# CognitiveAISystems/MAPF-GPT

Measured on AMD Instinct MI355X. Metric: agent-steps/s (env+obs+GPT fwd), higher is better.
Workload: dtype f16x3

## Files before the change

mapf_gpt_amd/csrc/gpt_kernels_attn_tiles.h:

```cpp
#pragma once
#include "gpt_kernels_c256p.h"

namespace mgpt {
namespace fastk {

constexpr int kAttNvb1 = 10, kAttNvb2 = 6;

__device__ unsigned long long g_attn_fallbacks = 0;

template <class T, int NP, int KROW, int VROW, int HS>
__device__ __forceinline__ void attention_exact_tiles(unsigned kr_addr, unsigned vr_addr, const u32x4 (&qf)[2][2], float sc2, f32x16 &o, float &l_run)
{
    float m_run, zero;
    asm volatile("v_mov_b32 %0, 0xff800000\n\tv_mov_b32 %1, 0" : "=v"(m_run), "=v"(zero));
    l_run = zero;
#pragma unroll
    for (int g = 0; g < 16; g++) o[g] = zero;
{
    u32x4 kf[2][2], vf[2][2];
    auto load_k = [&](int kt) {
        const unsigned a = kr_addr + (unsigned)kt * (32 * KROW);
        asm volatile("ds_read_b128 %0, %1" : "=v"(kf[0][0]) : "v"(a) : "memory");
        asm volatile("ds_read_b128 %0, %1 offset:32" : "=v"(kf[1][0]) : "v"(a) : "memory");
        if (NP == 2) {
            asm volatile("ds_read_b128 %0, %1 offset:%2" : "=v"(kf[0][1]) : "v"(a), "n"(kT * KROW) : "memory");
            asm volatile("ds_read_b128 %0, %1 offset:%2" : "=v"(kf[1][1]) : "v"(a), "n"(kT * KROW + 32) : "memory");
        } else { kf[0][1] = kf[0][0]; kf[1][1] = kf[1][0]; }
    };
    load_k(0);
#pragma unroll 1
    for (int kt = 0; kt < kT / 32; kt++) {
        f32x16 sc;
#pragma unroll
        for (int g = 0; g < 16; g++) sc[g] = 0.f;
        asm volatile("s_waitcnt lgkmcnt(0)" ::: "memory");
        __builtin_amdgcn_sched_barrier(0);
#pragma unroll
        for (int ks = 0; ks < 2; ks++) sc = mma<T, NP>(kf[ks], qf[ks], sc);
        __builtin_amdgcn_sched_barrier(0);
        {
            const unsigned a = vr_addr + (unsigned)kt * 64;
            asm volatile("ds_read_b128 %0, %1" : "=v"(vf[0][0]) : "v"(a) : "memory");
            asm volatile("ds_read_b128 %0, %1 offset:32" : "=v"(vf[1][0]) : "v"(a) : "memory");
            if (NP == 2) {
                asm volatile("ds_read_b128 %0, %1 offset:%2" : "=v"(vf[0][1]) : "v"(a), "n"(HS * VROW) : "memory");
                asm volatile("ds_read_b128 %0, %1 offset:%2" : "=v"(vf[1][1]) : "v"(a), "n"(HS * VROW + 32) : "memory");
            } else { vf[0][1] = vf[0][0]; vf[1][1] = vf[1][0]; }
        }
        if (kt + 1 < kT / 32) load_k(kt + 1);
        float mx = sc[0];
#pragma unroll
        for (int g = 1; g < 16; g++) mx = fmaxf(mx, sc[g]);
        mx = other_half_max(mx);
        if (__builtin_amdgcn_ballot_w64(mx > m_run) != 0) {
            const float m_new = fmaxf(m_run, mx);
            const float alpha = __builtin_amdgcn_exp2f((m_run - m_new) * sc2);
            l_run *= alpha;
#pragma unroll
            for (int g = 0; g < 16; g++) o[g] *= alpha;
            m_run = m_new;
        }
        const float nm = -m_run * sc2;
        float psum = 0.f;
#pragma unroll
        for (int g = 0; g < 16; g++) {
            sc[g] = __builtin_amdgcn_exp2f(fmaf(sc[g], sc2, nm));
            psum += sc[g];
        }
        l_run += other_half_sum(psum);
        u32x4 pf[2][2];
#pragma unroll
        for (int mm = 0; mm < 2; mm++) pack_octet<T, NP>(sc, mm, pf[mm]);
        if (kt + 1 < kT / 32) asm volatile("s_waitcnt lgkmcnt(%0)" ::"n"(2 * NP) : "memory");
        else asm volatile("s_waitcnt lgkmcnt(0)" ::: "memory");
        __builtin_amdgcn_sched_barrier(0);
#pragma unroll
        for (int mm = 0; mm < 2; mm++) o = mma<T, NP>(vf[mm], pf[mm], o);
    }
}
}

template <class T, int NP, int KROW, int VROW, int HS>
__device__ __forceinline__ void attention_tiles(unsigned kr_addr, unsigned vr_addr, const u32x4 (&qf)[2][2], int lane, f32x16 &o, float &l_run)
{
    using I0 = std::integral_constant<int, 0>;
    using I1 = std::integral_constant<int, 1>;

    u32x4 kf[2][2], vf[2][2], pf[2][2];
    f32x16 sA, sB;
    constexpr int NM = NP == 2 ? 3 : 1;
    auto amfma = [&](u32x4 a, u32x4 b2, f32x16 c) { return T::mfma(a, b2, c); };
    auto amma = [&](const u32x4 (&a)[2], const u32x4 (&b2)[2], f32x16 c) {
        if (NP == 2) { c = amfma(a[1], b2[0], c); c = amfma(a[0], b2[1], c); }
        return amfma(a[0], b2[0], c);
    };
    auto load_k = [&](auto kt_c) {
        constexpr int off = decltype(kt_c)::value * (32 * KROW);
        asm volatile("ds_read_b128 %0, %1 offset:%2" : "=v"(kf[0][0]) : "v"(kr_addr), "n"(off) : "memory");
        asm volatile("ds_read_b128 %0, %1 offset:%2" : "=v"(kf[1][0]) : "v"(kr_addr), "n"(off + 32) : "memory");
        if (NP == 2) {
            asm volatile("ds_read_b128 %0, %1 offset:%2" : "=v"(kf[0][1]) : "v"(kr_addr), "n"(off + kT * KROW) : "memory");
            asm volatile("ds_read_b128 %0, %1 offset:%2" : "=v"(kf[1][1]) : "v"(kr_addr), "n"(off + kT * KROW + 32) : "memory");
        } else { kf[0][1] = kf[0][0]; kf[1][1] = kf[1][0]; }
    };
    auto load_v = [&](auto kt_c, auto mm_c) {
        constexpr int off = decltype(kt_c)::value * 64 + decltype(mm_c)::value * 32, mm = decltype(mm_c)::value;
        asm volatile("ds_read_b128 %0, %1 offset:%2" : "=v"(vf[mm][0]) : "v"(vr_addr), "n"(off) : "memory");
        if (NP == 2) asm volatile("ds_read_b128 %0, %1 offset:%2" : "=v"(vf[mm][1]) : "v"(vr_addr), "n"(off + HS * VROW) : "memory");
        else vf[mm][1] = vf[mm][0];
    };
    auto lgkm = [&](auto n_c) {
        asm volatile("s_waitcnt lgkmcnt(%0)" ::"n"(decltype(n_c)::value) : "memory");
        __builtin_amdgcn_sched_barrier(0);
    };
    auto place = [&](auto nmf_c, auto nv_c) {
#pragma unroll
        for (int n = 0; n < decltype(nmf_c)::value; n++) {
            __builtin_amdgcn_sched_group_barrier(0x008, 1, 0);
            __builtin_amdgcn_sched_group_barrier(0x002, decltype(nv_c)::value, 0);
        }
        __builtin_amdgcn_sched_group_barrier(0x002, 64, 0);
        __builtin_amdgcn_sched_barrier(0);
    };
    using LK = std::integral_constant<int, 2 * NP>;
    using LV = std::integral_constant<int, NP>;
    load_k(I0{});
    lgkm(I0{});
#pragma unroll
    for (int g = 0; g < 16; g++) sA[g] = 0.f;
#pragma unroll
    for (int ks = 0; ks < 2; ks++) sA = amma(kf[ks], qf[ks], sA);
    __builtin_amdgcn_sched_barrier(0);
    load_k(I1{});
    f32x16 nmb;
    {
        float mx = sA[0];
#pragma unroll
        for (int g = 1; g < 16; g++) mx = fmaxf(mx, sA[g]);
        const float nm = -other_half_max(mx);
#pragma unroll
        for (int g = 0; g < 16; g++) { nmb[g] = nm; sA[g] += nm; }
    }
    float l_part = 0.f;
    auto tile = [&](auto kt_c, f32x16 &cur, f32x16 &nxt) {
        constexpr int kt = decltype(kt_c)::value;
        constexpr bool FIRSTT = kt == 0, LASTT = kt == kT / 32 - 1, HAS2 = kt + 2 < kT / 32;
        if constexpr (!FIRSTT) {
            lgkm(std::integral_constant<int, LASTT ? 0 : LK::value>{});
            o = amma(vf[1], pf[1], o);
#pragma unroll
            for (int g = 0; g < 4; g++) {
                cur[g] = __builtin_amdgcn_exp2f(cur[g]);
                l_part += cur[g];
            }
            place(std::integral_constant<int, NM>{}, std::integral_constant<int, 4>{});
            asm volatile("" : "+v"(o));
        }
        load_v(kt_c, I0{});
        if constexpr (!LASTT) {
            lgkm(LV{});
            nxt = amma(kf[0], qf[0], nmb);
            nxt = amma(kf[1], qf[1], nxt);
        }
#pragma unroll
        for (int g = FIRSTT ? 0 : 4; g < 16; g++) {
            cur[g] = __builtin_amdgcn_exp2f(cur[g]);
            l_part += cur[g];
        }
        pack_octet<T, NP>(cur, 0, pf[0]);
        place(std::integral_constant<int, LASTT ? 0 : 2 * NM>{}, std::integral_constant<int, kAttNvb1>{});
        if constexpr (!LASTT) asm volatile("" : "+v"(nxt));
        load_v(kt_c, I1{});
        lgkm(LV{});
        if constexpr (FIRSTT) {
#pragma unroll
            for (int g = 0; g < 16; g++) o[g] = 0.f;
        }
        o = amma(vf[0], pf[0], o);
        pack_octet<T, NP>(cur, 1, pf[1]);
        place(std::integral_constant<int, NM>{}, std::integral_constant<int, kAttNvb2>{});
        asm volatile("" : "+v"(o));
        if constexpr (HAS2) load_k(std::integral_constant<int, HAS2 ? kt + 2 : 0>{});
    };
    using K0 = std::integral_constant<int, 0>; using K1 = std::integral_constant<int, 1>; using K2 = std::integral_constant<int, 2>; using K3 = std::integral_constant<int, 3>;
    using K4 = std::integral_constant<int, 4>; using K5 = std::integral_constant<int, 5>; using K6 = std::integral_constant<int, 6>; using K7 = std::integral_constant<int, 7>;
    static_assert(kT / 32 == 8, "eight key tiles");
    tile(K0{}, sA, sB); tile(K1{}, sB, sA); tile(K2{}, sA, sB); tile(K3{}, sB, sA);
    tile(K4{}, sA, sB); tile(K5{}, sB, sA); tile(K6{}, sA, sB); tile(K7{}, sB, sA);
    lgkm(I0{});
    o = amma(vf[1], pf[1], o);
    __builtin_amdgcn_sched_barrier(0);
    l_run = other_half_sum(l_part);
    if (__builtin_amdgcn_ballot_w64(!(l_part < 60000.0f)) != 0) {
        if (lane == 0) atomicAdd(&g_attn_fallbacks, 1ull);
        attention_exact_tiles<T, NP, KROW, VROW, HS>(kr_addr, vr_addr, qf, 1.0f, o, l_run);
    }
}

}
}
```

mapf_gpt_amd/csrc/gpt_kernels_c256b.h:

```cpp
#pragma once
#include "gpt_kernels_c256p.h"
#include "gpt_kernels_attn_tiles.h"

namespace mgpt {
namespace fastk {

constexpr int kA256oProjSteps = 16;
constexpr int kA256oPeriod = 8 * kA256StepsPerHead + kA256oProjSteps;


template <class T, int NP>
__global__ __launch_bounds__(256) void pack_attn256q_kernel(const float *__restrict__ w_attn, const float *__restrict__ gain,
                                                            const float *__restrict__ w_proj, uint16_t *__restrict__ out,
                                                            float scale_a, float scale_p)
{
    constexpr int C = 256, NH = 8, QKV = NH * kA256StepsPerHead;
    const int64_t gid = (int64_t)blockIdx.x * 256 + threadIdx.x;
    if (gid >= (int64_t)kA256oPeriod * 8 * 64) return;
    const int lane = (int)(gid & 63), ms = (int)((gid >> 6) & 7), G = (int)(gid >> 9);
    const int rho = lane & 15, qk = lane >> 4;
    float v[8];
    if (G < QKV) {
        const int head = G / kA256StepsPerHead, st = G - head * kA256StepsPerHead;
        int which, kb, dim;
        if (st < 4) {
            const int cc = 4 * st + (ms >> 1), ug = ms & 1, rq = rho >> 2;
            kb = cc >> 1; which = cc & 1;
            const int blk = which == 0 ? 2 * (rq & 1) + (rq >> 1) : rq;
            dim = 8 * blk + 4 * ug + (rho & 3);
        } else { which = 2; kb = 4 * (st - 4) + (ms >> 1); dim = 16 * (ms & 1) + rho; }
        const float *row = w_attn + (size_t)(which * C + head * 32 + dim) * C;
#pragma unroll
        for (int e = 0; e < 8; e++) {
            const int col = 32 * kb + 8 * qk + e;
            v[e] = row[col] * gain[col] * scale_a;
        }
    } else {
        const int s = G - QKV, tt = s >> 2, j = s & 3;
        const int cc = 4 * j + (ms >> 1), kb = cc >> 1, fgl = 2 * (cc & 1) + (ms & 1);
        const float *row = w_proj + (size_t)(64 * tt + 16 * fgl + rho) * C;
#pragma unroll
        for (int e = 0; e < 8; e++) {
            const int col = 32 * kb + (e & 3) + 8 * (2 * (qk & 1) + (e >> 2)) + 4 * (qk >> 1);
            v[e] = row[col] * scale_p;
        }
    }
    u32x2 h0, l0, h1, l1;
    split4<T, NP>(v, h0, l0);
    split4<T, NP>(v + 4, h1, l1);
    u32x4 hi, lo;
    hi[0] = h0[0]; hi[1] = h0[1]; hi[2] = h1[0]; hi[3] = h1[1];
    lo[0] = l0[0]; lo[1] = l0[1]; lo[2] = l1[0]; lo[3] = l1[1];
    uint16_t *dst = out + (((size_t)G * 8 + ms) * NP) * 512 + (size_t)lane * 8;
    *reinterpret_cast<u32x4 *>(dst) = hi;
    if (NP == 2) *reinterpret_cast<u32x4 *>(dst + 512) = lo;
}

template <int NP> constexpr int kL0TabHeadBytes = 192 * NP;
template <int NP> constexpr int kL0TabEntryBytes = 8 * kL0TabHeadBytes<NP>;
template <class T, int NP, bool EMB = false, int TAB = 0>
__global__ __launch_bounds__(512, 2) void attn256q_kernel(float *__restrict__ x, const uint16_t *__restrict__ wstream, float inv_scale,
                                                          float scale_log2e, float inv_proj, unsigned char *__restrict__ spill,
                                                          int n_rows, const unsigned char *__restrict__ tokens = nullptr,
                                                          const float *__restrict__ etab = nullptr, unsigned char *__restrict__ table = nullptr)
{
    static_assert(TAB == 0 || (TAB == 1 && EMB) || (TAB == 2 && !EMB), "table modes");
    constexpr int HB = kL0TabHeadBytes<NP>, ENT = kL0TabEntryBytes<NP>;
    constexpr int C = 256, KS = 16, NH = 8, HS = 32, NW = 8;
    static_assert(NP == 2 || NP == 1, "planes");
    constexpr int MS = 8;
    constexpr int STEP = MS * NP * 1024;
    constexpr int NSLOT = 5;
    constexpr int PW = MS * NP / NW;
    constexpr int KROW = 80, VROW = 528;
    constexpr int NSPILL = 2 * NP;
    constexpr int NYLD = 14 * NP;
    static_assert(PW >= 1, "a wave moves at least one piece per step");
    extern __shared__ __attribute__((aligned(16))) unsigned char smem[];
    const int tid = threadIdx.x, lane = tid & 63;
    const int wave = __builtin_amdgcn_readfirstlane(tid >> 6);
    const int tok0 = wave * 32;
    const unsigned lane16 = (unsigned)lane * 16u;
    const unsigned lds0 = (unsigned)(size_t)smem + lane16;
    const unsigned sK = (unsigned)(size_t)smem + NSLOT * STEP, sV = sK + NP * kT * KROW;
    constexpr int PERIOD = TAB == 2 ? kA256oProjSteps : kA256oPeriod;
    const unsigned char *wbase = reinterpret_cast<const unsigned char *>(wstream) + (size_t)(wave * PW) * 1024 +
                                 (TAB == 2 ? (size_t)(kA256oPeriod - kA256oProjSteps) * STEP : 0);
    unsigned char *sp_wave = spill + ((size_t)blockIdx.x * NW + wave) * (size_t)(14 * NP * 1024);
    const int n_mine = n_rows > (int)blockIdx.x ? (n_rows - 1 - (int)blockIdx.x) / (int)gridDim.x + 1 : 0;
    if (n_mine == 0) return;

    int r_issue = 0;
    int slot_cur = 0, slot_prev = NSLOT - 1;
    unsigned cur_addr = 0, nxt_addr = 0;
    auto issue = [&](int slot) {
        const unsigned char *src = wbase + (size_t)r_issue * STEP;
        unsigned char *dst = smem + (size_t)slot * STEP + (size_t)(wave * PW) * 1024;
#pragma unroll
        for (int i = 0; i < PW; i++) dma_piece(src + lane16, dst, std::integral_constant<int, 0>{}, i);
        r_issue = r_issue + 1 == PERIOD ? 0 : r_issue + 1;
    };
#pragma unroll
    for (int G = 0; G < NSLOT - 1; G++) issue(G);
    auto sync_wait = [&](auto pending_c) {
        vm_wait<decltype(pending_c)::value>();
        __builtin_amdgcn_s_barrier();
    };
    int slot_refill = 0;
    auto sync_issue = [&]() {
        issue(slot_prev);
        const int slot_next = slot_cur + 1 == NSLOT ? 0 : slot_cur + 1;
        cur_addr = lds0 + (unsigned)slot_cur * STEP;
        nxt_addr = lds0 + (unsigned)slot_next * STEP;
        slot_prev = slot_cur;
        slot_cur = slot_next;
    };
    u32x4 wb[2][2][2];
    auto chunk_wait = [&]() {
        asm volatile("s_waitcnt lgkmcnt(0)" ::: "memory");
        __builtin_amdgcn_sched_barrier(0);
    };
    auto chunk_read = [&](auto c_c, auto next_c, auto n_c) {
        constexpr int c = decltype(c_c)::value, n = decltype(n_c)::value;
        if constexpr (n < 2 * NP) {
            constexpr int fr = n / NP, pl = n % NP;
            if constexpr (c < 3) lds_frag(cur_addr, std::integral_constant<int, ((2 * c + 2 + fr) * NP + pl) * 1024>{}, wb[(c + 1) & 1][fr][pl]);
            else if constexpr (decltype(next_c)::value) lds_frag(nxt_addr, std::integral_constant<int, (fr * NP + pl) * 1024>{}, wb[0][fr][pl]);
            if constexpr (NP == 1 && (c < 3 || decltype(next_c)::value)) wb[(c + 1) & 1][fr][1] = wb[(c + 1) & 1][fr][0];
            __builtin_amdgcn_sched_barrier(0);
        }
    };
    using I0 = std::integral_constant<int, 0>;
    using I1 = std::integral_constant<int, 1>;
    using I2 = std::integral_constant<int, 2>;
    using I3 = std::integral_constant<int, 3>;
    auto mma4 = [&](const u32x4 (&w0)[2], const u32x4 (&w1)[2], const u32x4 (&x0)[2], const u32x4 (&x1)[2], f32x16 &blk, auto swap_c, auto first_c, auto &&behind) {
        constexpr bool SW = decltype(swap_c)::value, FIRST = decltype(first_c)::value;
        auto one = [&](const u32x4 &w, const u32x4 &xx, auto s_c) {
            if constexpr (SW) mm16<T>(xx, w, blk, s_c); else mm16<T>(w, xx, blk, s_c);
        };
        auto onez = [&](const u32x4 &w, const u32x4 &xx, auto s_c) {
            if constexpr (!FIRST) one(w, xx, s_c);
            else if constexpr (SW) mm16z<T>(xx, w, blk, s_c);
            else mm16z<T>(w, xx, blk, s_c);
        };
        if (NP == 2) {
            onez(w0[1], x0[0], I0{}); behind(I0{}); onez(w1[1], x0[0], I1{}); behind(I1{}); onez(w0[1], x1[0], I2{}); behind(I2{}); onez(w1[1], x1[0], I3{}); behind(I3{});
            one(w0[0], x0[1], I0{}); behind(std::integral_constant<int, 4>{}); one(w1[0], x0[1], I1{}); behind(std::integral_constant<int, 5>{});
            one(w0[0], x1[1], I2{}); one(w1[0], x1[1], I3{});
            one(w0[0], x0[0], I0{}); one(w1[0], x0[0], I1{}); one(w0[0], x1[0], I2{}); one(w1[0], x1[0], I3{});
        } else {
            onez(w0[0], x0[0], I0{}); behind(I0{}); onez(w1[0], x0[0], I1{}); behind(I1{}); onez(w0[0], x1[0], I2{}); behind(I2{}); onez(w1[0], x1[0], I3{});
        }
    };
    auto chunk_body = [&](auto c_c, auto next_c, auto &&mm) {
        chunk_wait();
        constexpr bool REFILL = false;
        constexpr int N_REFILL = NP == 2 ? 5 : 2, N_LAST = REFILL ? N_REFILL : 2 * NP - 1, NMF = NP == 2 ? 12 : 4;
        mm([&](auto n_c) {
            constexpr int n = decltype(n_c)::value;
            if constexpr (n < 2 * NP) { __builtin_amdgcn_sched_barrier(0); chunk_read(c_c, next_c, n_c); }
            else if constexpr (REFILL && n == N_REFILL) { __builtin_amdgcn_sched_barrier(0); issue(slot_refill); __builtin_amdgcn_sched_barrier(0); }
        });
#pragma unroll
        for (int n = 0; n < NMF - 1 - N_LAST; n++) __builtin_amdgcn_sched_group_barrier(0x008, 1, 0);
        __builtin_amdgcn_sched_barrier(0);
    };
    const float q_units = scale_log2e * inv_scale, k_units = inv_scale;

    u32x4 xn[KS][2];

    f32x16 qa, ka;
    auto step_pair = [&](auto j_c, auto pending_c, auto &&after_barrier, auto next_c) {
        constexpr int j = decltype(j_c)::value;
        sync_wait(pending_c);
        after_barrier();
        sync_issue();
        auto chunk = [&](auto c_c) {
            constexpr int c = decltype(c_c)::value;
            constexpr int cc = 4 * j + c, kb = cc >> 1;
            chunk_body(c_c, next_c, [&](auto &&behind) {
                using F = std::integral_constant<bool, (cc < 2)>;
                if constexpr ((cc & 1) == 0) mma4(wb[c & 1][0], wb[c & 1][1], xn[kb], xn[8 + kb], qa, std::false_type{}, F{}, behind);
                else mma4(wb[c & 1][0], wb[c & 1][1], xn[kb], xn[8 + kb], ka, std::false_type{}, F{}, behind);
            });
            asm volatile("" : "+v"(qa), "+v"(ka));
        };
        chunk(I0{}); chunk(I1{}); chunk(I2{}); chunk(I3{});
    };
    auto nothing = [&]() {};
    asm volatile("s_waitcnt vmcnt(0)" ::: "memory");
    __builtin_amdgcn_s_barrier();
    nxt_addr = lds0;
    using P4 = std::integral_constant<int, PW * (NSLOT - 3)>;
    using P4S = std::integral_constant<int, PW * (NSLOT - 3) + NSPILL>;

#pragma unroll 1
    for (int k = 0; k < n_mine; k++) {
        const int64_t b = (int64_t)blockIdx.x + (int64_t)k * gridDim.x;
        unsigned char *xw = reinterpret_cast<unsigned char *>(x + (b * kT + tok0) * C);
        unsigned ent0 = 0, ent1 = 0;
        if constexpr (TAB == 2) {
            unsigned l16p = lane16;
            asm volatile("" : "+v"(l16p));
            const unsigned char *tk = tokens + b * kT + tok0;
            const unsigned tt_p = (l16p >> 4) & 15u;
            unsigned id0, id1;
            asm volatile("global_load_ubyte %0, %1, %2" : "=v"(id0) : "v"(tt_p), "s"(tk) : "memory");
            asm volatile("global_load_ubyte %0, %1, %2 offset:16" : "=v"(id1) : "v"(tt_p), "s"(tk) : "memory");
            asm volatile("s_waitcnt vmcnt(0)" : "+v"(id0), "+v"(id1) : : "memory");
            ent0 = ((unsigned)tok0 + tt_p) * 67u + id0;
            ent1 = ((unsigned)tok0 + 16u + tt_p) * 67u + id1;
        } else {
            unsigned l16p = lane16;
            asm volatile("" : "+v"(l16p));
            const unsigned xoff_p = (l16p >> 8) * 1024 + ((l16p >> 4) & 15u) * 32;
            f32x4 xr[32];
            if constexpr (EMB) {
                const unsigned char *tk = tokens + b * kT + tok0;
                const unsigned tt_p = (l16p >> 4) & 15u;
                unsigned id0, id1;
                asm volatile("global_load_ubyte %0, %1, %2" : "=v"(id0) : "v"(tt_p), "s"(tk) : "memory");
                asm volatile("global_load_ubyte %0, %1, %2 offset:16" : "=v"(id1) : "v"(tt_p), "s"(tk) : "memory");
                asm volatile("s_waitcnt vmcnt(0)" : "+v"(id0), "+v"(id1) : : "memory");
                const unsigned q32 = (l16p >> 8) * 32u;
                const unsigned ve0 = (((unsigned)tok0 + tt_p) * 67u + id0) * 1024u + q32;
                const unsigned ve1 = (((unsigned)tok0 + 16u + tt_p) * 67u + id1) * 1024u + q32;
                const unsigned char *eb = reinterpret_cast<const unsigned char *>(etab);
#pragma unroll
                for (int i = 0; i < 32; i++) {
                    if (((i >> 1) & 1) == 0)
                        asm volatile("global_load_dwordx4 %0, %1, %2 offset:%3" : "=v"(xr[2 * (i >> 2) + (i & 1)]) : "v"(ve0), "s"(eb), "n"((i >> 2) * 128 + (i & 1) * 16) : "memory");
                    else
                        asm volatile("global_load_dwordx4 %0, %1, %2 offset:%3" : "=v"(xr[2 * (8 + (i >> 2)) + (i & 1)]) : "v"(ve1), "s"(eb), "n"((i >> 2) * 128 + (i & 1) * 16) : "memory");
                }
            } else {
#pragma unroll
            for (int i = 0; i < 32; i++) {
                const unsigned char *xq = xw + (i >> 2) * 4096;
                asm volatile("global_load_dwordx4 %0, %1, %2 offset:%3" : "=v"(xr[2 * (8 * ((i >> 1) & 1) + (i >> 2)) + (i & 1)]) : "v"(xoff_p), "s"(xq), "n"(((i >> 1) & 1) * 512 + (i & 1) * 16) : "memory");
            }
            }
            asm volatile("s_waitcnt vmcnt(0)" : "+v"(xr[0]), "+v"(xr[1]), "+v"(xr[2]), "+v"(xr[3]), "+v"(xr[4]), "+v"(xr[5]), "+v"(xr[6]), "+v"(xr[7]) : : "memory");
            asm volatile("" : "+v"(xr[8]), "+v"(xr[9]), "+v"(xr[10]), "+v"(xr[11]), "+v"(xr[12]), "+v"(xr[13]), "+v"(xr[14]), "+v"(xr[15]));
            asm volatile("" : "+v"(xr[16]), "+v"(xr[17]), "+v"(xr[18]), "+v"(xr[19]), "+v"(xr[20]), "+v"(xr[21]), "+v"(xr[22]), "+v"(xr[23]));
            asm volatile("" : "+v"(xr[24]), "+v"(xr[25]), "+v"(xr[26]), "+v"(xr[27]), "+v"(xr[28]), "+v"(xr[29]), "+v"(xr[30]), "+v"(xr[31]));
            if constexpr (EMB) {
#pragma unroll
                for (int i = 0; i < 32; i++) {
                    const unsigned char *xq = xw + (i >> 2) * 4096;
                    asm volatile("global_store_dwordx4 %0, %1, %2 offset:%3\n\ts_nop 1" ::"v"(xoff_p), "v"(xr[2 * (8 * ((i >> 1) & 1) + (i >> 2)) + (i & 1)]), "s"(xq), "n"(((i >> 1) & 1) * 512 + (i & 1) * 16) : "memory");
                }
            }
            float rstd[2];
#pragma unroll
            for (int tg = 0; tg < 2; tg++) {
                float sm = 0.f;
#pragma unroll
                for (int i = 0; i < 16; i++) sm += (xr[16 * tg + i][0] + xr[16 * tg + i][1]) + (xr[16 * tg + i][2] + xr[16 * tg + i][3]);
                const float mean = permlane_fold4(sm) * (1.0f / (float)C);
                float qv = 0.f;
#pragma unroll
                for (int i = 0; i < 16; i++)
#pragma unroll
                    for (int e = 0; e < 4; e++) { const float d = xr[16 * tg + i][e] - mean; xr[16 * tg + i][e] = d; qv = fmaf(d, d, qv); }
                rstd[tg] = rsqrtf(permlane_fold4(qv) * (1.0f / (float)C) + 1e-5f);
            }
#pragma unroll
            for (int ks = 0; ks < KS; ks++) {
                float v0[4], v1[4];
#pragma unroll
                for (int e = 0; e < 4; e++) { v0[e] = xr[2 * ks][e] * rstd[ks >> 3]; v1[e] = xr[2 * ks + 1][e] * rstd[ks >> 3]; }
                u32x2 h0, l0, h1, l1;
                split4p<T, NP>(v0, h0, l0);
                split4p<T, NP>(v1, h1, l1);
                xn[ks][0][0] = h0[0]; xn[ks][0][1] = h0[1]; xn[ks][0][2] = h1[0]; xn[ks][0][3] = h1[1];
                xn[ks][1][0] = l0[0]; xn[ks][1][1] = l0[1]; xn[ks][1][2] = l1[0]; xn[ks][1][3] = l1[1];
                if ((ks & 1) == 1) __builtin_amdgcn_sched_barrier(0);
            }
        }
        if constexpr (TAB != 2) {
            lds_pair<NP>(nxt_addr, I0{}, wb[0][0]);
            lds_pair<NP>(nxt_addr, I1{}, wb[0][1]);
        }

        auto head = [&](int hd, auto last_c) {
            constexpr bool LASTH = decltype(last_c)::value;
            unsigned l16 = lane16;
            asm volatile("" : "+v"(l16));
            const unsigned rr = (l16 >> 4) & 31u, hh = l16 >> 9;
            const unsigned kr_addr = sK + rr * KROW + hh * 16;
            const unsigned vr_addr = sV + rr * VROW + hh * 16;
            const unsigned tt = (l16 >> 4) & 15u, qq = l16 >> 8;
            const unsigned kw_addr = sK + ((unsigned)tok0 + tt) * KROW + qq * 16;
            const unsigned vw_addr = sV + tt * VROW + (unsigned)wave * 64 + (qq & 1u) * 16 + (qq >> 1) * 8;
            asm volatile("" : "=v"(qa), "=v"(ka));
            step_pair(I0{}, P4S{}, nothing, std::true_type{});
            step_pair(I1{}, P4S{}, nothing, std::true_type{});
            step_pair(I2{}, P4S{}, nothing, std::true_type{});
            step_pair(I3{}, P4{}, nothing, std::true_type{});
            u32x4 qf[2][2];
#pragma unroll
            for (int g = 0; g < 16; g++) { qa[g] *= q_units; ka[g] *= k_units; }
#pragma unroll
            for (int tg = 0; tg < 2; tg++) pack_octet<T, NP>(qa, tg, qf[tg]);
#pragma unroll
            for (int pl = 0; pl < NP; pl++)
#pragma unroll
                for (int wd = 0; wd < 4; wd++) { unsigned a = qf[0][pl][wd], b2 = qf[1][pl][wd]; row_swap(a, b2); qf[0][pl][wd] = a; qf[1][pl][wd] = b2; }
            if (NP == 1) { qf[0][1] = qf[0][0]; qf[1][1] = qf[1][0]; }
            if constexpr (TAB == 1) {
                const unsigned voff = (((unsigned)tok0 + rr) * 67u * ENT) + (unsigned)b * ENT + (unsigned)hd * HB + hh * (32 * NP);
#pragma unroll
                for (int ks = 0; ks < 2; ks++)
#pragma unroll
                    for (int pl = 0; pl < NP; pl++)
                        asm volatile("global_store_dwordx4 %0, %1, %2 offset:%3\n\ts_nop 1" ::"v"(voff), "v"(qf[ks][pl]), "s"(table), "n"((ks * NP + pl) * 16) : "memory");
            }
            {
                u32x4 kp[2][2];
#pragma unroll
                for (int tg = 0; tg < 2; tg++) pack_octet<T, NP>(ka, tg, kp[tg]);
#pragma unroll
                for (int tg = 0; tg < 2; tg++)
#pragma unroll
                    for (int pl = 0; pl < NP; pl++)
                        asm volatile("ds_write_b128 %0, %1 offset:%2" ::"v"(kw_addr), "v"(kp[tg][pl]), "n"(pl * kT * KROW + tg * 16 * KROW) : "memory");
                if constexpr (TAB == 1) {
#pragma unroll
                    for (int tg = 0; tg < 2; tg++) {
                        const unsigned voff = (((unsigned)tok0 + 16u * tg + tt) * 67u * ENT) + (unsigned)b * ENT + (unsigned)hd * HB + 64 * NP + qq * (16 * NP);
#pragma unroll
                        for (int pl = 0; pl < NP; pl++)
                            asm volatile("global_store_dwordx4 %0, %1, %2 offset:%3\n\ts_nop 1" ::"v"(voff), "v"(kp[tg][pl]), "s"(table), "n"(pl * 16) : "memory");
                    }
                }
            }
            f32x16 va;
            auto step_v = [&](auto j_c, auto next_c) {
                constexpr int j = decltype(j_c)::value;
                sync_wait(P4{});
                sync_issue();
                auto chunk = [&](auto c_c) {
                    constexpr int c = decltype(c_c)::value;
                    constexpr int kb = 4 * j + c;
                    chunk_body(c_c, next_c, [&](auto &&behind) { mma4(wb[c & 1][0], wb[c & 1][1], xn[kb], xn[8 + kb], va, std::true_type{}, std::integral_constant<bool, kb == 0>{}, behind); });
                    asm volatile("" : "+v"(va));
                };
                chunk(I0{}); chunk(I1{}); chunk(I2{}); chunk(I3{});
            };
            step_v(I0{}, std::true_type{});
            step_v(I1{}, std::false_type{});
            if constexpr (LASTH) {
#pragma unroll
                for (int hh2 = 0; hh2 < 7; hh2++)
#pragma unroll
                    for (int tg = 0; tg < 2; tg++)
#pragma unroll
                        for (int pl = 0; pl < NP; pl++) {
                            const unsigned char *p = sp_wave + (size_t)hh2 * (size_t)(2 * NP * 1024);
                            asm volatile("global_load_dwordx4 %0, %1, %2 offset:%3" : "=v"(xn[8 * tg + hh2][pl]) : "v"(lane16), "s"(p), "n"((tg * NP + pl) * 1024) : "memory");
                        }
            }
            {
#pragma unroll
                for (int sl = 0; sl < 4; sl++) {
                    u32x2 vp[2];
                    unsigned a0, b0, a1, b1;
                    split2p<T, NP>(va[4 * sl], va[4 * sl + 1], a0, b0);
                    split2p<T, NP>(va[4 * sl + 2], va[4 * sl + 3], a1, b1);
                    vp[0][0] = a0; vp[0][1] = a1; vp[1][0] = b0; vp[1][1] = b1;
#pragma unroll
                    for (int pl = 0; pl < NP; pl++)
                        asm volatile("ds_write_b64 %0, %1 offset:%2" ::"v"(vw_addr), "v"(vp[pl]), "n"(pl * HS * VROW + (sl & 1) * 16 * VROW + (sl >> 1) * 32) : "memory");
                    if constexpr (TAB == 1) {
#pragma unroll
                        for (int i = 0; i < 4; i++) {
                            const unsigned voff = (((unsigned)tok0 + 16u * (sl >> 1) + 4u * qq + i) * 67u * ENT) + (unsigned)b * ENT + (unsigned)hd * HB + 128 * NP +
                                                  (16u * (sl & 1) + tt) * 2u;
#pragma unroll
                            for (int pl = 0; pl < NP; pl++) {
                                if (i & 1) asm volatile("global_store_short_d16_hi %0, %1, %2 offset:%3" ::"v"(voff), "v"(vp[pl][i >> 1]), "s"(table), "n"(pl * 64) : "memory");
                                else asm volatile("global_store_short %0, %1, %2 offset:%3" ::"v"(voff), "v"(vp[pl][i >> 1]), "s"(table), "n"(pl * 64) : "memory");
                            }
                        }
                    }
                }
            }
            if constexpr (TAB == 1) asm volatile("s_waitcnt vmcnt(0)" ::: "memory");
            asm volatile("s_waitcnt lgkmcnt(0)" ::: "memory");
            __builtin_amdgcn_s_barrier();

            f32x16 o;
            float l_run = 0.f;
            attention_tiles<T, NP, KROW, VROW, HS>(kr_addr, vr_addr, qf, lane, o, l_run);
            lds_pair<NP>(nxt_addr, I0{}, wb[0][0]);
            lds_pair<NP>(nxt_addr, I1{}, wb[0][1]);
            {
                const float inv = inv_scale / l_run;
#pragma unroll
                for (int g = 0; g < 16; g++) o[g] *= inv;
#pragma unroll
                for (int g = 0; g < 8; g++) { float a = o[g], b2 = o[8 + g]; asm volatile("s_nop 1\n\tv_permlane16_swap_b32 %0, %1" : "+v"(a), "+v"(b2)); o[g] = a; o[8 + g] = b2; }
                if constexpr (LASTH) {
                    pack_octet<T, NP>(o, 0, xn[7]);
                    pack_octet<T, NP>(o, 1, xn[15]);
                } else {
                    u32x4 yp[2][2];
                    pack_octet<T, NP>(o, 0, yp[0]);
                    pack_octet<T, NP>(o, 1, yp[1]);
                    unsigned char *p = sp_wave + (size_t)hd * (size_t)(2 * NP * 1024);
#pragma unroll
                    for (int kk = 0; kk < 2; kk++)
#pragma unroll
                        for (int pl = 0; pl < NP; pl++)
                            asm volatile("global_store_dwordx4 %0, %1, %2 offset:%3\n\ts_nop 1" ::"v"(lane16), "v"(yp[kk][pl]), "s"(p), "n"((kk * NP + pl) * 1024) : "memory");
                }
            }
        };
        auto head_t = [&](int hd) {
            unsigned l16 = lane16;
            asm volatile("" : "+v"(l16));
            const unsigned rr = (l16 >> 4) & 31u, hh = l16 >> 9;
            const unsigned kr_addr = sK + rr * KROW + hh * 16;
            const unsigned vr_addr = sV + rr * VROW + hh * 16;
            const unsigned tt = (l16 >> 4) & 15u, qq = l16 >> 8;
            const unsigned kw_addr = sK + ((unsigned)tok0 + tt) * KROW + qq * 16;
            const unsigned vt_addr = sV + qq * 8 * VROW + (unsigned)wave * 64 + (((tt >> 2) & 1u) * 8 + ((tt >> 3) & 1u) * 4 + (tt & 3u)) * 2;
            const unsigned hoff = (unsigned)hd * HB;
            const unsigned e0 = ent0 * ENT + hoff, e1 = ent1 * ENT + hoff;
            const unsigned qoff = ((qq & 1u) ? e1 : e0) + hh * (32 * NP);
            u32x4 qf[2][2], kp[2][2], vq[2][2];
#pragma unroll
            for (int ks = 0; ks < 2; ks++)
#pragma unroll
                for (int pl = 0; pl < NP; pl++)
                    asm volatile("global_load_dwordx4 %0, %1, %2 offset:%3" : "=v"(qf[ks][pl]) : "v"(qoff), "s"(table), "n"((ks * NP + pl) * 16) : "memory");
#pragma unroll
            for (int tg = 0; tg < 2; tg++) {
                const unsigned ko = (tg ? e1 : e0) + qq * (16 * NP), vo = (tg ? e1 : e0) + qq * 16;
#pragma unroll
                for (int pl = 0; pl < NP; pl++) {
                    asm volatile("global_load_dwordx4 %0, %1, %2 offset:%3" : "=v"(kp[tg][pl]) : "v"(ko), "s"(table), "n"(64 * NP + pl * 16) : "memory");
                    asm volatile("global_load_dwordx4 %0, %1, %2 offset:%3" : "=v"(vq[tg][pl]) : "v"(vo), "s"(table), "n"(128 * NP + pl * 64) : "memory");
                }
            }
            __builtin_amdgcn_s_barrier();
            if constexpr (NP == 2)
                asm volatile("s_waitcnt vmcnt(0)" : "+v"(qf[0][0]), "+v"(qf[0][1]), "+v"(qf[1][0]), "+v"(qf[1][1]), "+v"(kp[0][0]), "+v"(kp[0][1]), "+v"(kp[1][0]), "+v"(kp[1][1]),
                             "+v"(vq[0][0]), "+v"(vq[0][1]), "+v"(vq[1][0]), "+v"(vq[1][1]) : : "memory");
            else
                asm volatile("s_waitcnt vmcnt(0)" : "+v"(qf[0][0]), "+v"(qf[1][0]), "+v"(kp[0][0]), "+v"(kp[1][0]), "+v"(vq[0][0]), "+v"(vq[1][0]) : : "memory");
            if (NP == 1) { qf[0][1] = qf[0][0]; qf[1][1] = qf[1][0]; }
#pragma unroll
            for (int tg = 0; tg < 2; tg++)
#pragma unroll
                for (int pl = 0; pl < NP; pl++) {
                    asm volatile("ds_write_b128 %0, %1 offset:%2" ::"v"(kw_addr), "v"(kp[tg][pl]), "n"(pl * kT * KROW + tg * 16 * KROW) : "memory");
#pragma unroll
                    for (int j = 0; j < 8; j++) {
                        if (j & 1) asm volatile("ds_write_b16_d16_hi %0, %1 offset:%2" ::"v"(vt_addr), "v"(vq[tg][pl][j >> 1]), "n"(pl * HS * VROW + j * VROW + tg * 32) : "memory");
                        else asm volatile("ds_write_b16 %0, %1 offset:%2" ::"v"(vt_addr), "v"(vq[tg][pl][j >> 1]), "n"(pl * HS * VROW + j * VROW + tg * 32) : "memory");
                    }
                }
            asm volatile("s_waitcnt lgkmcnt(0)" ::: "memory");
            __builtin_amdgcn_s_barrier();
            f32x16 o;
            float l_run = 0.f;
            attention_tiles<T, NP, KROW, VROW, HS>(kr_addr, vr_addr, qf, lane, o, l_run);
            const float inv = inv_scale / l_run;
#pragma unroll
            for (int g = 0; g < 16; g++) o[g] *= inv;
#pragma unroll
            for (int g = 0; g < 8; g++) { float a = o[g], b2 = o[8 + g]; asm volatile("s_nop 1\n\tv_permlane16_swap_b32 %0, %1" : "+v"(a), "+v"(b2)); o[g] = a; o[8 + g] = b2; }
#pragma unroll
            for (int k2 = 0; k2 < 7; k2++)
#pragma unroll
                for (int pl = 0; pl < NP; pl++) { xn[k2][pl] = xn[k2 + 1][pl]; xn[8 + k2][pl] = xn[9 + k2][pl]; }
            pack_octet<T, NP>(o, 0, xn[7]);
            pack_octet<T, NP>(o, 1, xn[15]);
        };
        if constexpr (TAB == 2) {
#pragma unroll 1
            for (int hd = 0; hd < NH; hd++) head_t(hd);
            lds_pair<NP>(nxt_addr, I0{}, wb[0][0]);
            lds_pair<NP>(nxt_addr, I1{}, wb[0][1]);
        } else {
#pragma unroll 1
            for (int hd = 0; hd < NH - 1; hd++) head(hd, std::false_type{});
            head(NH - 1, std::true_type{});
        }

        auto tail = [&](int t, auto first_c, auto last_c) {
            constexpr bool FIRST = decltype(first_c)::value, LASTT = decltype(last_c)::value;
            asm volatile("" : "=v"(qa), "=v"(ka));
            unsigned l16t = lane16;
            asm volatile("" : "+v"(l16t));
            const unsigned xoff_t = (l16t >> 9) * 1024 + ((l16t >> 4) & 15u) * 32 + ((l16t >> 8) & 1u) * 16;
            const unsigned qq_t = l16t >> 8;
            f32x4 xs[4][2];
            unsigned char *xp = xw + (size_t)t * 8192;
            constexpr int OTHERS = 8;
            auto requests = [&]() {
                if constexpr (TAB == 2) {
                    const unsigned r0 = ent0 * (C * 4) + (unsigned)t * 256 + qq_t * 16, r1 = ent1 * (C * 4) + (unsigned)t * 256 + qq_t * 16;
                    const unsigned char *eb = reinterpret_cast<const unsigned char *>(etab);
#pragma unroll
                    for (int fgl = 0; fgl < 4; fgl++) {
                        asm volatile("global_load_dwordx4 %0, %1, %2 offset:%3" : "=v"(xs[fgl][0]) : "v"(r0), "s"(eb), "n"(fgl * 64) : "memory");
                        asm volatile("global_load_dwordx4 %0, %1, %2 offset:%3" : "=v"(xs[fgl][1]) : "v"(r1), "s"(eb), "n"(fgl * 64) : "memory");
                    }
                    return;
                }
#pragma unroll
                for (int fgl = 0; fgl < 4; fgl++)
#pragma unroll
                    for (int tg = 0; tg < 2; tg++)
                        asm volatile("global_load_dwordx4 %0, %1, %2 offset:%3" : "=v"(xs[fgl][tg]) : "v"(xoff_t), "s"(xp + (fgl >> 1) * 4096), "n"((fgl & 1) * 2048 + tg * 512) : "memory");
            };
            step_pair(I0{}, std::integral_constant<int, 2 * PW + (FIRST ? (TAB == 2 ? 0 : NYLD) : 8)>{}, requests, std::true_type{});
            step_pair(I1{}, std::integral_constant<int, 2 * PW + 8 + OTHERS>{}, nothing, std::true_type{});
            step_pair(I2{}, std::integral_constant<int, 2 * PW + 8 + OTHERS>{}, nothing, std::true_type{});
            step_pair(I3{}, P4{}, nothing, std::integral_constant<bool, !LASTT>{});
            asm volatile("s_waitcnt vmcnt(%[n])" : "+v"(xs[0][0]), "+v"(xs[0][1]), "+v"(xs[1][0]), "+v"(xs[1][1]), "+v"(xs[2][0]), "+v"(xs[2][1]), "+v"(xs[3][0]), "+v"(xs[3][1])
                         : [n] "n"(4 * PW) : "memory");
#pragma unroll
            for (int fgl = 0; fgl < 4; fgl++)
#pragma unroll
                for (int tg = 0; tg < 2; tg++) {
                    f32x4 v;
#pragma unroll
                    for (int e = 0; e < 4; e++) v[e] = fmaf((fgl < 2 ? qa : ka)[4 * (2 * tg + (fgl & 1)) + e], inv_proj, xs[fgl][tg][e]);
                    asm volatile("global_store_dwordx4 %0, %1, %2 offset:%3\n\ts_nop 1" ::"v"(xoff_t), "v"(v), "s"(xp + (fgl >> 1) * 4096), "n"((fgl & 1) * 2048 + tg * 512) : "memory");
                }
        };
        {
            asm volatile("s_waitcnt vmcnt(0)" : "+v"(xn[0][0]), "+v"(xn[0][1]), "+v"(xn[1][0]), "+v"(xn[1][1]), "+v"(xn[2][0]), "+v"(xn[2][1]), "+v"(xn[3][0]), "+v"(xn[3][1]),
                         "+v"(xn[4][0]), "+v"(xn[4][1]), "+v"(xn[5][0]), "+v"(xn[5][1]), "+v"(xn[6][0]), "+v"(xn[6][1]) : : "memory");
            asm volatile("" : "+v"(xn[8][0]), "+v"(xn[8][1]), "+v"(xn[9][0]), "+v"(xn[9][1]), "+v"(xn[10][0]), "+v"(xn[10][1]), "+v"(xn[11][0]), "+v"(xn[11][1]),
                         "+v"(xn[12][0]), "+v"(xn[12][1]), "+v"(xn[13][0]), "+v"(xn[13][1]), "+v"(xn[14][0]), "+v"(xn[14][1]));
            asm volatile("" : "+v"(xn[7][0]), "+v"(xn[7][1]), "+v"(xn[15][0]), "+v"(xn[15][1]));
        }
        tail(0, std::true_type{}, std::false_type{});
#pragma unroll 1
        for (int t = 1; t < 3; t++) tail(t, std::false_type{}, std::false_type{});
        tail(3, std::false_type{}, std::true_type{});
    }
    asm volatile("s_waitcnt vmcnt(0)" ::: "memory");
}

}
}
```

Measured before the change: 127,600.

## Prefetch next head's Q/K/V global loads during current head's attention tiles

In the TAB==2 per-head loop, the global loads of Q, K and V for the next head are issued from inside the current head's attention at the start of the last tile, so their latency overlaps that tile's compute. Before, each head issued its loads only after the previous head finished. A hook parameter is added to attention_tiles for this. The rare fallback path, which would otherwise clobber the in-flight registers, first drains them, reloads Q and then reissues the prefetch. The cost is more live VGPRs (register pressure) plus extra complexity in the fallback.

```diff
diff --git a/mapf_gpt_amd/csrc/gpt_kernels_attn_tiles.h b/mapf_gpt_amd/csrc/gpt_kernels_attn_tiles.h
--- a/mapf_gpt_amd/csrc/gpt_kernels_attn_tiles.h
+++ b/mapf_gpt_amd/csrc/gpt_kernels_attn_tiles.h
@@ -80,9 +80,16 @@
 }
 }
 
-template <class T, int NP, int KROW, int VROW, int HS>
-__device__ __forceinline__ void attention_tiles(unsigned kr_addr, unsigned vr_addr, const u32x4 (&qf)[2][2], int lane, f32x16 &o, float &l_run)
+struct NoAhead {
+    __device__ __forceinline__ void request() const {}
+    __device__ __forceinline__ void reload_q(u32x4 (&)[2][2]) const {}
+};
+template <class Req, class Reload> struct AheadOf { Req request; Reload reload_q; };
+
+template <class T, int NP, int KROW, int VROW, int HS, class Ahead = NoAhead>
+__device__ __forceinline__ void attention_tiles(unsigned kr_addr, unsigned vr_addr, const u32x4 (&qf)[2][2], int lane, f32x16 &o, float &l_run, Ahead ahead = Ahead{})
 {
+    constexpr bool AHEAD = !std::is_same<Ahead, NoAhead>::value;
     using I0 = std::integral_constant<int, 0>;
     using I1 = std::integral_constant<int, 1>;
 
@@ -145,6 +152,10 @@
     auto tile = [&](auto kt_c, f32x16 &cur, f32x16 &nxt) {
         constexpr int kt = decltype(kt_c)::value;
         constexpr bool FIRSTT = kt == 0, LASTT = kt == kT / 32 - 1, HAS2 = kt + 2 < kT / 32;
+        if constexpr (AHEAD && LASTT) {
+            ahead.request();
+            __builtin_amdgcn_sched_barrier(0);
+        }
         if constexpr (!FIRSTT) {
             lgkm(std::integral_constant<int, LASTT ? 0 : LK::value>{});
             o = amma(vf[1], pf[1], o);
@@ -193,7 +204,13 @@
     l_run = other_half_sum(l_part);
     if (__builtin_amdgcn_ballot_w64(!(l_part < 60000.0f)) != 0) {
         if (lane == 0) atomicAdd(&g_attn_fallbacks, 1ull);
-        attention_exact_tiles<T, NP, KROW, VROW, HS>(kr_addr, vr_addr, qf, 1.0f, o, l_run);
+        if constexpr (AHEAD) {
+            u32x4 q2[2][2];
+            ahead.reload_q(q2);
+            attention_exact_tiles<T, NP, KROW, VROW, HS>(kr_addr, vr_addr, q2, 1.0f, o, l_run);
+            ahead.request();
+        } else
+            attention_exact_tiles<T, NP, KROW, VROW, HS>(kr_addr, vr_addr, qf, 1.0f, o, l_run);
     }
 }
 
diff --git a/mapf_gpt_amd/csrc/gpt_kernels_c256b.h b/mapf_gpt_amd/csrc/gpt_kernels_c256b.h
--- a/mapf_gpt_amd/csrc/gpt_kernels_c256b.h
+++ b/mapf_gpt_amd/csrc/gpt_kernels_c256b.h
@@ -418,7 +418,31 @@
                 }
             }
         };
-        auto head_t = [&](int hd) {
+        u32x4 tq[2][2], tk[2][2], tv[2][2];
+        auto quads_t = [&](int hd) {
+            unsigned l16 = lane16;
+            asm volatile("" : "+v"(l16));
+            const unsigned hh = l16 >> 9, qq = l16 >> 8;
+            const unsigned hoff = (unsigned)hd * HB;
+            const unsigned e0 = ent0 * ENT + hoff, e1 = ent1 * ENT + hoff;
+            const unsigned qoff = ((qq & 1u) ? e1 : e0) + hh * (32 * NP);
+#pragma unroll
+            for (int ks = 0; ks < 2; ks++)
+#pragma unroll
+                for (int pl = 0; pl < NP; pl++)
+                    asm volatile("global_load_dwordx4 %0, %1, %2 offset:%3" : "=v"(tq[ks][pl]) : "v"(qoff), "s"(table), "n"((ks * NP + pl) * 16) : "memory");
+#pragma unroll
+            for (int tg = 0; tg < 2; tg++) {
+                const unsigned ko = (tg ? e1 : e0) + qq * (16 * NP), vo = (tg ? e1 : e0) + qq * 16;
+#pragma unroll
+                for (int pl = 0; pl < NP; pl++) {
+                    asm volatile("global_load_dwordx4 %0, %1, %2 offset:%3" : "=v"(tk[tg][pl]) : "v"(ko), "s"(table), "n"(64 * NP + pl * 16) : "memory");
+                    asm volatile("global_load_dwordx4 %0, %1, %2 offset:%3" : "=v"(tv[tg][pl]) : "v"(vo), "s"(table), "n"(128 * NP + pl * 64) : "memory");
+                }
+            }
+        };
+        auto head_t = [&](int hd, auto more_c) {
+            constexpr bool MORE = decltype(more_c)::value;
             unsigned l16 = lane16;
             asm volatile("" : "+v"(l16));
             const unsigned rr = (l16 >> 4) & 31u, hh = l16 >> 9;
@@ -427,30 +451,17 @@
             const unsigned tt = (l16 >> 4) & 15u, qq = l16 >> 8;
             const unsigned kw_addr = sK + ((unsigned)tok0 + tt) * KROW + qq * 16;
             const unsigned vt_addr = sV + qq * 8 * VROW + (unsigned)wave * 64 + (((tt >> 2) & 1u) * 8 + ((tt >> 3) & 1u) * 4 + (tt & 3u)) * 2;
-            const unsigned hoff = (unsigned)hd * HB;
-            const unsigned e0 = ent0 * ENT + hoff, e1 = ent1 * ENT + hoff;
-            const unsigned qoff = ((qq & 1u) ? e1 : e0) + hh * (32 * NP);
-            u32x4 qf[2][2], kp[2][2], vq[2][2];
-#pragma unroll
-            for (int ks = 0; ks < 2; ks++)
-#pragma unroll
-                for (int pl = 0; pl < NP; pl++)
-                    asm volatile("global_load_dwordx4 %0, %1, %2 offset:%3" : "=v"(qf[ks][pl]) : "v"(qoff), "s"(table), "n"((ks * NP + pl) * 16) : "memory");
-#pragma unroll
-            for (int tg = 0; tg < 2; tg++) {
-                const unsigned ko = (tg ? e1 : e0) + qq * (16 * NP), vo = (tg ? e1 : e0) + qq * 16;
-#pragma unroll
-                for (int pl = 0; pl < NP; pl++) {
-                    asm volatile("global_load_dwordx4 %0, %1, %2 offset:%3" : "=v"(kp[tg][pl]) : "v"(ko), "s"(table), "n"(64 * NP + pl * 16) : "memory");
-                    asm volatile("global_load_dwordx4 %0, %1, %2 offset:%3" : "=v"(vq[tg][pl]) : "v"(vo), "s"(table), "n"(128 * NP + pl * 64) : "memory");
-                }
-            }
             __builtin_amdgcn_s_barrier();
             if constexpr (NP == 2)
-                asm volatile("s_waitcnt vmcnt(0)" : "+v"(qf[0][0]), "+v"(qf[0][1]), "+v"(qf[1][0]), "+v"(qf[1][1]), "+v"(kp[0][0]), "+v"(kp[0][1]), "+v"(kp[1][0]), "+v"(kp[1][1]),
-                             "+v"(vq[0][0]), "+v"(vq[0][1]), "+v"(vq[1][0]), "+v"(vq[1][1]) : : "memory");
+                asm volatile("s_waitcnt vmcnt(0)" : "+v"(tq[0][0]), "+v"(tq[0][1]), "+v"(tq[1][0]), "+v"(tq[1][1]), "+v"(tk[0][0]), "+v"(tk[0][1]), "+v"(tk[1][0]), "+v"(tk[1][1]),
+                             "+v"(tv[0][0]), "+v"(tv[0][1]), "+v"(tv[1][0]), "+v"(tv[1][1]) : : "memory");
             else
-                asm volatile("s_waitcnt vmcnt(0)" : "+v"(qf[0][0]), "+v"(qf[1][0]), "+v"(kp[0][0]), "+v"(kp[1][0]), "+v"(vq[0][0]), "+v"(vq[1][0]) : : "memory");
+                asm volatile("s_waitcnt vmcnt(0)" : "+v"(tq[0][0]), "+v"(tq[1][0]), "+v"(tk[0][0]), "+v"(tk[1][0]), "+v"(tv[0][0]), "+v"(tv[1][0]) : : "memory");
+            u32x4 qf[2][2], kp[2][2], vq[2][2];
+#pragma unroll
+            for (int i = 0; i < 2; i++)
+#pragma unroll
+                for (int pl = 0; pl < NP; pl++) { qf[i][pl] = tq[i][pl]; kp[i][pl] = tk[i][pl]; vq[i][pl] = tv[i][pl]; }
             if (NP == 1) { qf[0][1] = qf[0][0]; qf[1][1] = qf[1][0]; }
 #pragma unroll
             for (int tg = 0; tg < 2; tg++)
@@ -467,7 +478,36 @@
             __builtin_amdgcn_s_barrier();
             f32x16 o;
             float l_run = 0.f;
-            attention_tiles<T, NP, KROW, VROW, HS>(kr_addr, vr_addr, qf, lane, o, l_run);
+            auto quads_end = [&]() {
+                if constexpr (NP == 2)
+                    asm volatile("" : "=v"(tq[0][0]), "=v"(tq[0][1]), "=v"(tq[1][0]), "=v"(tq[1][1]), "=v"(tk[0][0]), "=v"(tk[0][1]), "=v"(tk[1][0]), "=v"(tk[1][1]),
+                                 "=v"(tv[0][0]), "=v"(tv[0][1]), "=v"(tv[1][0]), "=v"(tv[1][1]));
+                else
+                    asm volatile("" : "=v"(tq[0][0]), "=v"(tq[1][0]), "=v"(tk[0][0]), "=v"(tk[1][0]), "=v"(tv[0][0]), "=v"(tv[1][0]));
+            };
+            auto request_next = [&]() {
+                if constexpr (MORE) quads_t(hd + 1);
+                else quads_end();
+            };
+            auto reload_q = [&](u32x4 (&q2)[2][2]) {
+                if constexpr (MORE) {
+                    if constexpr (NP == 2)
+                        asm volatile("s_waitcnt vmcnt(0)" : "+v"(tq[0][0]), "+v"(tq[0][1]), "+v"(tq[1][0]), "+v"(tq[1][1]), "+v"(tk[0][0]), "+v"(tk[0][1]), "+v"(tk[1][0]),
+                                     "+v"(tk[1][1]), "+v"(tv[0][0]), "+v"(tv[0][1]), "+v"(tv[1][0]), "+v"(tv[1][1]) : : "memory");
+                    else
+                        asm volatile("s_waitcnt vmcnt(0)" : "+v"(tq[0][0]), "+v"(tq[1][0]), "+v"(tk[0][0]), "+v"(tk[1][0]), "+v"(tv[0][0]), "+v"(tv[1][0]) : : "memory");
+                    quads_end();
+                }
+                const unsigned qoff = ((qq & 1u) ? ent1 : ent0) * ENT + (unsigned)hd * HB + hh * (32 * NP);
+#pragma unroll
+                for (int ks = 0; ks < 2; ks++)
+#pragma unroll
+                    for (int pl = 0; pl < NP; pl++)
+                        asm volatile("global_load_dwordx4 %0, %1, %2 offset:%3" : "=v"(q2[ks][pl]) : "v"(qoff), "s"(table), "n"((ks * NP + pl) * 16) : "memory");
+                if constexpr (NP == 2) asm volatile("s_waitcnt vmcnt(0)" : "+v"(q2[0][0]), "+v"(q2[0][1]), "+v"(q2[1][0]), "+v"(q2[1][1]) : : "memory");
+                else { asm volatile("s_waitcnt vmcnt(0)" : "+v"(q2[0][0]), "+v"(q2[1][0]) : : "memory"); q2[0][1] = q2[0][0]; q2[1][1] = q2[1][0]; }
+            };
+            attention_tiles<T, NP, KROW, VROW, HS>(kr_addr, vr_addr, qf, lane, o, l_run, AheadOf<decltype(request_next), decltype(reload_q)>{request_next, reload_q});
             const float inv = inv_scale / l_run;
 #pragma unroll
             for (int g = 0; g < 16; g++) o[g] *= inv;
@@ -481,8 +521,10 @@
             pack_octet<T, NP>(o, 1, xn[15]);
         };
         if constexpr (TAB == 2) {
+            quads_t(0);
 #pragma unroll 1
-            for (int hd = 0; hd < NH; hd++) head_t(hd);
+            for (int hd = 0; hd < NH - 1; hd++) head_t(hd, std::true_type{});
+            head_t(NH - 1, std::false_type{});
             lds_pair<NP>(nxt_addr, I0{}, wb[0][0]);
             lds_pair<NP>(nxt_addr, I1{}, wb[0][1]);
         } else {
```

Result: no change. 127,900, median of 6 (+0.2%).
